# cloneofsimo/paint-with-words-sd

Measured on AMD Instinct MI355X. Metric: 512x512 images/sec (30 steps, CFG) SD1.5+PwW, higher is better.
Workload: dtype bf16

## Files before the change

__graft_entry__.py:

```python
import os
import sys

REPO = os.path.dirname(os.path.abspath(__file__))
PKG = os.path.join(REPO, "paint-with-words-sd_amd")
for p in (PKG, REPO, os.path.join(REPO, "tests")):
    if p not in sys.path:
        sys.path.insert(0, p)


def build():
    import build as pww_build
    lib = pww_build.build_lib(verbose=False)
    exe = pww_build.build_native_check()
    long_lib = pww_build.build_long()
    scope_lib = pww_build.build_scope()
    import pww_hip
    import paint_with_words
    handle = pww_hip.load_library()
    missing = [n for n in pww_hip.EXPORTS if not hasattr(handle, n)]
    assert not missing, "libpww_hip.so lacks %s" % missing
    from pww_hip import _lib
    long_handle = _lib.load_long()
    missing = [n for n in _lib.LONG_EXPORTS if not hasattr(long_handle, n)]
    assert not missing, "libpww_hip_long.so lacks %s" % missing
    scope_handle = _lib.load_scope()
    assert scope_handle is not None, "%s was not built" % scope_lib
    missing = [n for n in _lib.SCOPE_EXPORTS if not hasattr(scope_handle, n)]
    assert not missing, "libpww_hip_scope.so lacks %s" % missing
    print("built %s (ABI %d), %s (ABI %d), %s (ABI %d) and %s" % (lib, handle.pww_version(), long_lib, long_handle.pww_long_version(),
                                                                  scope_lib, scope_handle.pww_scope_version(), exe))


def smoke():
    import math
    import numpy as np
    import torch
    import pww_hip
    from oracle import pww_oracle as O
    import pww_cases as cases

    assert torch.cuda.is_available(), "smoke() needs a HIP device"
    dev = torch.device("cuda:0")
    print("device arch:", pww_hip.device_arch())

    case = cases.make_attention_case("sd15_n1024")
    dtype = torch.float16
    mod = case["attn_cross"].to(dev, dtype)
    hidden = case["hidden"].to(dev, dtype)
    wf = lambda w, sigma, qk: 0.4 * w * math.log(1 + sigma) * qk.max()
    ctx = {"CONTEXT_TENSOR": case["ctx"].to(dev, dtype), "CROSS_ATTENTION_WEIGHT_1024": case["w"].to(dev),
           "SIGMA": torch.tensor(7.84), "WEIGHT_FUNCTION": wf}
    y = pww_hip.inj_forward(mod, hidden, ctx).float().cpu()
    mod_ref = case["attn_cross"].to("cpu", dtype).float()
    ctx_ref = {"CONTEXT_TENSOR": case["ctx"].to(dtype).float(), "CROSS_ATTENTION_WEIGHT_1024": case["w"],
               "SIGMA": torch.tensor(7.84), "WEIGHT_FUNCTION": wf}
    ref = O.inj_forward(mod_ref, case["hidden"].to(dtype).float(), ctx_ref)
    err = (y - ref).abs().max().item() / ref.abs().max().item()
    print("cross-attention + PwW bias: max err / max|O| = %.3e" % err)
    assert err < 5e-3, err

    import paint_with_words as pw
    from PIL import Image
    tools = cases.build_tools("tiny", dtype=dtype, device=dev)
# ... 24 lines not shown
```

paint-with-words-sd_amd/build.py:

```python
import os
import subprocess
import sys

HERE = os.path.dirname(os.path.abspath(__file__))
REPO = os.path.dirname(HERE)
CSRC = os.path.join(HERE, "csrc")
LIB = os.path.join(HERE, "pww_hip", "libpww_hip.so")
LIB_EXPERIMENTS = os.path.join(HERE, "pww_hip", "libpww_hip_experiments.so")
LIB_LONG = os.path.join(HERE, "pww_hip", "libpww_hip_long.so")
LIB_SCOPE = os.path.join(HERE, "pww_hip", "libpww_hip_scope.so")
UNITS = [("pww_api.hip", [], ""), ("pww_attn.hip", [], ""), ("pww_cross.hip", [], ""), ("pww_cross_lean.hip", [], ""), ("pww_reduce.hip", [], ""),
         ("pww_mask.hip", [], ""), ("pww_qproj.hip", [], ""), ("pww_norm.hip", [], ""), ("pww_blocks.hip", [], ""), ("pww_conv.hip", [], ""), ("pww_probs.hip", [], ""),
         ("pww_attn_inst.hip", ["-DPWW_INST_F16"], ".f16"), ("pww_attn_inst.hip", ["-DPWW_INST_BF16"], ".bf16"),
         ("pww_cross_inst.hip", ["-DPWW_INST_F16", "-DPWW_INST_NW=2"], ".f16.nw2"), ("pww_cross_inst.hip", ["-DPWW_INST_F16", "-DPWW_INST_NW=4"], ".f16.nw4"),
         ("pww_cross_inst.hip", ["-DPWW_INST_BF16", "-DPWW_INST_NW=2"], ".bf16.nw2"), ("pww_cross_inst.hip", ["-DPWW_INST_BF16", "-DPWW_INST_NW=4"], ".bf16.nw4")]
EXPERIMENT_UNITS = [("pww_cross_out.hip", [], "")]
LONG_UNITS = [("pww_long.hip", ["-fvisibility=hidden"], "")]
LONG_HEADERS = ["pww_common.h", "pww_tile.h", "pww_attn_core.h", "pww_cross_tile.h", os.path.join(REPO, "include", "pww_hip.h"), os.path.join(REPO, "include", "pww_hip_long.h")]
SCOPE_UNITS = [("pww_scope.hip", ["-fvisibility=hidden"], "")]
SCOPE_HEADERS = ["pww_common.h", "pww_tile.h", "pww_attn_core.h", "pww_cross_tile.h", os.path.join(REPO, "include", "pww_hip.h"), os.path.join(REPO, "include", "pww_hip_scope.h")]
SOURCES = sorted({u[0] for u in UNITS + EXPERIMENT_UNITS})
HEADERS = ["pww_common.h", "pww_tile.h", "pww_attn_core.h", "pww_attn_kernel.h", "pww_cross_tile.h", "pww_cross_kernel.h", os.path.join(REPO, "include", "pww_hip.h")]
HIPCC = os.environ.get("HIPCC", "/opt/rocm/bin/hipcc")
FLAGS = ["--offload-arch=gfx950", "-O3", "-std=c++17", "-fPIC", "-Wall",
         "-Wno-unused-function", "-mllvm", "-amdgpu-kernarg-preload-count=16"]


PER_FILE_FLAGS = {"pww_mask.hip": ["-ffp-contract=off"]}


def _newer(target, deps):
    if not os.path.exists(target):
        return True
    t = os.path.getmtime(target)
    return any(os.path.getmtime(d) > t for d in deps)


def _deps():
    return ([os.path.join(CSRC, s) for s in SOURCES] + [h if os.path.isabs(h) else os.path.join(CSRC, h) for h in HEADERS] + [__file__])


def _build(lib, units, defines, objdir, verbose, jobs=None):
    os.makedirs(objdir, exist_ok=True)
    order = sorted(units, key=lambda u: {"pww_cross_inst.hip": 0, "pww_attn_inst.hip": 1, "pww_cross_lean.hip": 2}.get(u[0], 3))
    jobs = jobs or max(2, min(len(order), (os.cpu_count() or 4)))
    pending, running, objs = list(order), [], []
    while pending or running:
        while pending and len(running) < jobs:
            src, defs, suffix = pending.pop(0)
            o = os.path.join(objdir, src + suffix + ".o")
            objs.append(o)
            cmd = [HIPCC] + FLAGS + defines + defs + PER_FILE_FLAGS.get(src, []) + ["-c", os.path.join(CSRC, src), "-o", o]
            if verbose:
# ... 7 lines not shown
            raise RuntimeError("hipcc failed: %s\n%s" % (" ".join(cmd), out))
        if verbose and out.strip():
            print(out)
    subprocess.run([HIPCC, "--offload-arch=gfx950", "-shared", "-fPIC", "-s"] + sorted(objs) + ["-o", lib], check=True)
    return lib


def build_lib(force=False, verbose=False):
    if not force and not _newer(LIB, _deps()):
        return LIB
    return _build(LIB, UNITS, [], os.path.join(HERE, "build"), verbose)


def build_experiments(force=False, verbose=False):
    if not force and not _newer(LIB_EXPERIMENTS, _deps()):
        return LIB_EXPERIMENTS
    return _build(LIB_EXPERIMENTS, UNITS + EXPERIMENT_UNITS, ["-DPWW_EXPERIMENTS=1"], os.path.join(HERE, "build", "experiments"), verbose)


def build_long(force=False, verbose=False):
    deps = [os.path.join(CSRC, u[0]) for u in LONG_UNITS] + [h if os.path.isabs(h) else os.path.join(CSRC, h) for h in LONG_HEADERS] + [__file__]
    if not force and not _newer(LIB_LONG, deps):
        return LIB_LONG
    return _build(LIB_LONG, LONG_UNITS, [], os.path.join(HERE, "build", "long"), verbose)


def build_scope(force=False, verbose=False):
    deps = [os.path.join(CSRC, u[0]) for u in SCOPE_UNITS] + [h if os.path.isabs(h) else os.path.join(CSRC, h) for h in SCOPE_HEADERS] + [__file__]
    if not force and not _newer(LIB_SCOPE, deps):
        return LIB_SCOPE
    return _build(LIB_SCOPE, SCOPE_UNITS, [], os.path.join(HERE, "build", "scope"), verbose)


def _build_check(exe, lib, libname, defines, force):
    src = os.path.join(REPO, "tests", "native", "attn_check.cpp")
    if not force and not _newer(exe, [src, lib, os.path.join(REPO, "include", "pww_hip.h")]):
        return exe
    cmd = [HIPCC, "--offload-arch=gfx950", "-O2", "-std=c++17"] + defines + [src, "-o", exe, "-L" + os.path.dirname(lib), "-l" + libname,
                                                                              "-Wl,-rpath,$ORIGIN/../../paint-with-words-sd_amd/pww_hip"]
    subprocess.run(cmd, check=True)
    return exe


def build_native_check(force=False):
    return _build_check(os.path.join(REPO, "tests", "native", "attn_check"), build_lib(), "pww_hip", [], force)


def build_native_check_experiments(force=False):
    return _build_check(os.path.join(REPO, "tests", "native", "attn_check_experiments"), build_experiments(), "pww_hip_experiments", ["-DPWW_EXPERIMENTS=1"], force)


if __name__ == "__main__":
    force = "--force" in sys.argv
    print(build_lib(force=force, verbose=True))
    print(build_native_check(force=force))
    print(build_long(force=force, verbose=True))
    print(build_scope(force=force, verbose=True))
    if "--experiments" in sys.argv:
        print(build_experiments(force=force, verbose=True))
        print(build_native_check_experiments(force=force))
```

paint-with-words-sd_amd/pww_hip/_lib.py:

```python
import ctypes
import os

_HERE = os.path.dirname(os.path.abspath(__file__))
LIB_PATH = os.environ.get("PWW_HIP_LIB", os.path.join(_HERE, "libpww_hip.so"))
EXPERIMENTS_LIB_PATH = os.environ.get("PWW_HIP_EXPERIMENTS_LIB", os.path.join(_HERE, "libpww_hip_experiments.so"))

LONG_LIB_PATH = os.environ.get("PWW_HIP_LONG_LIB", os.path.join(_HERE, "libpww_hip_long.so"))

SCOPE_LIB_PATH = os.environ.get("PWW_HIP_SCOPE_LIB", os.path.join(_HERE, "libpww_hip_scope.so"))

PWW_OK, PWW_EINVAL, PWW_ENOTSUP, PWW_EHIP = 0, -22, -95, -5
MIN_VERSION = 126
DTYPE_F16, DTYPE_BF16 = 0, 1
LAYOUT_NCHW, LAYOUT_NHWC = 0, 1
ACT_NONE, ACT_SILU = 0, 1
MAX_HEAD_DIM = 160

EXPORTS = ("pww_version", "pww_has_experiments", "pww_last_error", "pww_device_arch", "pww_self_attn_fwd", "pww_cross_attn_fwd",
           "pww_cross_attn_fwd_stat", "pww_cross_attn_fwd_stat_ex",
           "pww_qk_reduce", "pww_mask_build", "pww_mask_build_rgb", "pww_mask_build_f32", "pww_resize_tokens", "pww_gauss_blur", "pww_inpaint_prep", "pww_cfg_combine", "pww_store_f32",
           "pww_workspace_bytes", "pww_profile_arm", "pww_profile_elapsed_us", "pww_profile_reset", "pww_debug_timeline", "pww_debug_path_counts",
           "pww_qproj_stat", "pww_qproj_parts", "pww_cross_attn_fwd_parts", "pww_mask_build_f32_levels", "pww_qk_parts", "pww_qk_parts_count",
           "pww_group_norm_fwd", "pww_group_norm_workspace_bytes", "pww_add_layer_norm", "pww_add_layer_norm_bias", "pww_geglu", "pww_bias_residual",
           "pww_conv3x3_workspace_bytes", "pww_conv3x3_fwd", "pww_cross_attn_probs")
EXPERIMENT_EXPORTS = ("pww_cross_attn_fwd_fused", "pww_cross_attn_fwd_fused_ex", "pww_cross_fused_workspace_bytes", "pww_cross_fused_state_bytes",
                      "pww_cross_attn_fwd_parts_out", "pww_cross_attn_out_supported")


LONG_EXPORTS = ("pww_long_version", "pww_long_last_error", "pww_long_qk_parts", "pww_long_qk_parts_count", "pww_long_cross_attn_fwd_parts",
                "pww_long_cross_attn_probs", "pww_long_profile_arm", "pww_long_profile_elapsed_us")
LONG_MIN_VERSION = 100
LONG_MIN_KEYS, LONG_MAX_KEYS = 129, 256


SCOPE_EXPORTS = ("pww_scope_version", "pww_scope_last_error", "pww_scope_head_parts_count", "pww_scope_head_parts", "pww_scope_cross_attn_fwd")
SCOPE_MIN_VERSION = 100
SCOPE_HEAD, SCOPE_ROW = 1, 2


class AttnDesc(ctypes.Structure):
    _fields_ = [("dtype", ctypes.c_int32), ("B", ctypes.c_int32), ("H", ctypes.c_int32), ("N", ctypes.c_int32),
                ("M", ctypes.c_int32), ("D", ctypes.c_int32),
                ("q_stride", ctypes.c_int64 * 3), ("k_stride", ctypes.c_int64 * 3),
                ("v_stride", ctypes.c_int64 * 3), ("o_stride", ctypes.c_int64 * 3),
                ("scale", ctypes.c_float), ("bias_stride", ctypes.c_int64 * 4)]


class CrossOpts(ctypes.Structure):
    _fields_ = [("size", ctypes.c_uint32), ("bias_cols", ctypes.c_int32), ("coeff_scalar_dev", ctypes.c_void_p),
                ("bias_compact", ctypes.c_void_p), ("col_idx", ctypes.c_void_p), ("R", ctypes.c_int32), ("gated_images", ctypes.c_int32),
                ("compact_stride", ctypes.c_int64 * 2), ("col_idx_stride", ctypes.c_int64)]


class QprojDesc(ctypes.Structure):
    _fields_ = [("dtype", ctypes.c_int32), ("B", ctypes.c_int32), ("N", ctypes.c_int32), ("Cin", ctypes.c_int32), ("H", ctypes.c_int32),
                ("D", ctypes.c_int32), ("M", ctypes.c_int32), ("x_stride", ctypes.c_int64 * 2), ("q_stride", ctypes.c_int64 * 2),
                ("k_stride", ctypes.c_int64 * 2)]


class GnDesc(ctypes.Structure):
    _fields_ = [("dtype", ctypes.c_int32), ("layout", ctypes.c_int32), ("B", ctypes.c_int32), ("C", ctypes.c_int32), ("HW", ctypes.c_int32),
                ("G", ctypes.c_int32), ("eps", ctypes.c_float), ("act", ctypes.c_int32), ("add_stride", ctypes.c_int32), ("_pad", ctypes.c_int32)]


class LnDesc(ctypes.Structure):
    _fields_ = [("dtype", ctypes.c_int32), ("C", ctypes.c_int32), ("rows", ctypes.c_int64), ("a_stride", ctypes.c_int64), ("x_stride", ctypes.c_int64),
                ("s_stride", ctypes.c_int64), ("y_stride", ctypes.c_int64), ("eps", ctypes.c_float), ("_pad", ctypes.c_int32)]


class ConvDesc(ctypes.Structure):
    _fields_ = [("size", ctypes.c_uint32), ("dtype", ctypes.c_int32), ("B", ctypes.c_int32), ("Hin", ctypes.c_int32), ("Win", ctypes.c_int32),
                ("Cin", ctypes.c_int32), ("Cout", ctypes.c_int32), ("stride", ctypes.c_int32), ("upsample", ctypes.c_int32), ("tile_n", ctypes.c_int32),
                ("splitk", ctypes.c_int32), ("_pad", ctypes.c_int32)]


class ProbsDesc(ctypes.Structure):
    _fields_ = [("size", ctypes.c_uint32), ("images", ctypes.c_int32), ("accumulate", ctypes.c_int32), ("weight", ctypes.c_float),
                ("out_stride", ctypes.c_int64 * 2)]


class Region(ctypes.Structure):
    _fields_ = [("r", ctypes.c_uint8), ("g", ctypes.c_uint8), ("b", ctypes.c_uint8), ("_pad", ctypes.c_uint8),
                ("strength", ctypes.c_float)]


class PwwHipError(RuntimeError):
    pass


_lib = None
_exp = None


def _bind(lib, experiments):
    vp, i32, i64, f32 = ctypes.c_void_p, ctypes.c_int32, ctypes.c_int64, ctypes.c_float
    lib.pww_version.restype = ctypes.c_int
    if lib.pww_version() // 100 != 1 or lib.pww_version() < MIN_VERSION:
        raise PwwHipError("libpww_hip ABI version %d.%02d is not 1.x >= 1.%02d (rebuild: python paint-with-words-sd_amd/build.py)"
                          % (lib.pww_version() // 100, lib.pww_version() % 100, MIN_VERSION % 100))
    lib.pww_last_error.restype = ctypes.c_char_p
    lib.pww_device_arch.argtypes = [ctypes.c_char_p, ctypes.c_size_t]
    lib.pww_self_attn_fwd.argtypes = [vp, vp, vp, vp, ctypes.POINTER(AttnDesc), vp]
    lib.pww_cross_attn_fwd.argtypes = [vp, vp, vp, vp, vp, vp, ctypes.POINTER(AttnDesc), vp]
    lib.pww_cross_attn_fwd_stat.argtypes = [vp, vp, vp, vp, vp, vp, i32, ctypes.c_double, f32, vp, ctypes.POINTER(AttnDesc), vp]
    lib.pww_cross_attn_fwd_stat_ex.argtypes = [vp, vp, vp, vp, vp, vp, i32, ctypes.c_double, f32, vp, ctypes.POINTER(AttnDesc),
                                               ctypes.POINTER(CrossOpts), vp]
# ... 145 lines not shown


def load_scope():
    global _scope
    if _scope is not None:
        return _scope
    if not os.path.isfile(SCOPE_LIB_PATH):
        return None
    hint = "(rebuild: python paint-with-words-sd_amd/build.py)"
    try:
        lib = ctypes.CDLL(SCOPE_LIB_PATH)
        lib.pww_scope_version.restype = ctypes.c_int
        version = lib.pww_scope_version()
    except (OSError, AttributeError) as e:
        raise PwwHipError("libpww_hip_scope.so at %s cannot be loaded: %s %s" % (SCOPE_LIB_PATH, e, hint))
    if version // 100 != 1 or version < SCOPE_MIN_VERSION:
        raise PwwHipError("libpww_hip_scope ABI version %d is not 1.x >= %d %s" % (version, SCOPE_MIN_VERSION, hint))
    missing = [n for n in SCOPE_EXPORTS if not hasattr(lib, n)]
    if missing:
        raise PwwHipError("libpww_hip_scope.so at %s lacks %s %s" % (SCOPE_LIB_PATH, missing, hint))
    vp, i32, f32 = ctypes.c_void_p, ctypes.c_int32, ctypes.c_float
    lib.pww_scope_last_error.restype = ctypes.c_char_p
    lib.pww_last_error = lib.pww_scope_last_error
    lib.pww_scope_head_parts_count.argtypes = [ctypes.POINTER(AttnDesc)]
    lib.pww_scope_head_parts_count.restype = ctypes.c_int32
    lib.pww_scope_head_parts.argtypes = [vp, vp, vp, ctypes.POINTER(AttnDesc), i32, vp, ctypes.c_size_t, vp]
    lib.pww_scope_head_parts.restype = ctypes.c_int
    lib.pww_scope_cross_attn_fwd.argtypes = [vp, vp, vp, vp, vp, i32, i32, f32, vp, ctypes.POINTER(AttnDesc), vp, i32, vp, ctypes.POINTER(CrossOpts), vp]
    lib.pww_scope_cross_attn_fwd.restype = ctypes.c_int
    _scope = lib
    return _scope


class experiments:

    def __enter__(self):
        global _lib
        load()
        self._prev = _lib
        _lib = load_experiments()
        return _lib

    def __exit__(self, *exc):
        global _lib
        _lib = self._prev
        return False


def check(rc, what, lib=None):
    if rc != PWW_OK:
        msg = (lib or load()).pww_last_error().decode("utf-8", "replace")
        raise PwwHipError("%s failed (rc=%d): %s" % (what, rc, msg))


def device_arch():
    buf = ctypes.create_string_buffer(64)
    check(load().pww_device_arch(buf, 64), "pww_device_arch")
    return buf.value.decode()
```

paint-with-words-sd_amd/pww_hip/blocks.py:

```python
import os
import types
import warnings

import torch
import torch.nn as nn
import torch.nn.functional as F

from . import ops

FUSED_NORM = os.environ.get("PWW_FUSED_NORM", "1") != "0"
BATCHED_TEMB = os.environ.get("PWW_BATCHED_TEMB", "1") != "0"
FOLD_CONV_BIAS = os.environ.get("PWW_FOLD_CONV_BIAS", "1") != "0"
CONV1X1_AS_LINEAR = os.environ.get("PWW_CONV1X1_AS_LINEAR", "1") != "0"
FUSE_FF_RESIDUAL = os.environ.get("PWW_FUSE_FF_RESIDUAL", "0") == "1"
CONV3X3 = os.environ.get("PWW_CONV3X3", "1") != "0"


_STATS = {k: [0, 0] for k in ("group_norm", "resnet_block", "transformer_block", "geglu", "conv1x1", "conv3x3")}
_UNRATED = ("conv1x1", "conv3x3")
_warned = set()


def stats():
    out = {k: {"fused": v[0], "declined": v[1]} for k, v in _STATS.items()}
    rated = [v for k, v in _STATS.items() if k not in _UNRATED]
    tot = sum(v[0] + v[1] for v in rated)
    out["hit_rate"] = (sum(v[0] for v in rated) / tot) if tot else None
    return out


def reset_stats():
    for v in _STATS.values():
        v[0] = v[1] = 0


def _count(op, fused, x=None, reason=None):
    _STATS[op][0 if fused else 1] += 1
    if not fused and FUSED_NORM and torch.is_tensor(x) and x.is_cuda and x.dtype in (torch.float16, torch.bfloat16):
        key = (op, reason)
        if key not in _warned:
            _warned.add(key)
            warnings.warn("pww_hip.blocks: %s call on a HIP %s tensor handed to the stock op (%s); pww_hip.blocks.stats() counts them"
                          % (op, str(x.dtype).split(".")[-1], reason or "shape / dtype the kernels do not take"), stacklevel=3)


def _why_not(x):
    if torch.is_autocast_enabled():
        return "torch.autocast is on: the norms run in fp32 there"
    if torch.is_grad_enabled() and torch.is_tensor(x) and x.requires_grad:
        return "autograd is recording: the kernels are forward-only"
    return None

# ... 176 lines not shown
    _STATS["conv1x1"][1] += 1
    return self._pww_orig_forward(x, *args, **kwargs)


def _is_conv1x1(m):
    return (isinstance(m, nn.Conv2d) and type(m).forward is nn.Conv2d.forward and m.kernel_size == (1, 1) and m.stride == (1, 1) and m.padding == (0, 0)
            and m.dilation == (1, 1) and m.groups == 1 and m.padding_mode == "zeros")


def _ln_takes(x, norm):
    return (FUSED_NORM and torch.is_tensor(x) and x.is_cuda and x.dtype in (torch.float16, torch.bfloat16) and x.dim() >= 2
            and len(norm.normalized_shape) == 1 and x.shape[-1] == norm.normalized_shape[0] and x.shape[-1] % 8 == 0 and x.shape[-1] <= 2048
            and (norm.weight is None or norm.weight.dtype == x.dtype) and not torch.is_autocast_enabled()
            and not (torch.is_grad_enabled() and (x.requires_grad or (norm.weight is not None and norm.weight.requires_grad))))


def _transformer_block_covered(m):
    return (all(isinstance(getattr(m, n, None), nn.LayerNorm) for n in ("norm1", "norm2", "norm3")) and hasattr(m, "attn1") and hasattr(m, "attn2")
            and hasattr(m, "ff") and not getattr(m, "only_cross_attention", False))


def _transformer_block_forward(self, *args, **kwargs):
    covered = 1 <= len(args) <= 2 and set(kwargs) <= {"context", "timestep"} and kwargs.get("timestep") is None and not (len(args) == 2 and "context" in kwargs)
    hidden_states = args[0] if args else None
    if not covered or not _ln_takes(hidden_states, self.norm1):
        _count("transformer_block", False, hidden_states, ("a call beyond (hidden_states, context, timestep=None): %d positional, keywords %s" % (len(args), sorted(kwargs)))
               if not covered else _why_not(hidden_states))
        return self._pww_orig_forward(*args, **kwargs)
    context = args[1] if len(args) == 2 else kwargs.get("context")
    _count("transformer_block", True)
    h = hidden_states
    n = ops.add_layer_norm(h, self.norm1.weight, self.norm1.bias, self.norm1.eps)
    h, n = ops.add_layer_norm(h, self.norm2.weight, self.norm2.bias, self.norm2.eps, a=self.attn1(n))
    lin = _ff_output_linear(self.ff) if FUSE_FF_RESIDUAL else None
    if lin is not None and lin.weight.dtype == h.dtype:
        h, n = ops.add_layer_norm(h, self.norm3.weight, self.norm3.bias, self.norm3.eps, a=self.attn2(n, context=context), post_bias=lin.bias)
        g = self.ff.net[0](n)
        return torch.addmm(h.reshape(-1, h.shape[-1]), g.reshape(-1, g.shape[-1]), lin.weight.t()).view(h.shape)
    h, n = ops.add_layer_norm(h, self.norm3.weight, self.norm3.bias, self.norm3.eps, a=self.attn2(n, context=context))
    return self.ff(n) + h


def _ff_output_linear(ff):
    net = getattr(ff, "net", None)
    if net is None or len(net) != 3 or type(ff).__name__ != "FeedForward" or "forward" in ff.__dict__:
        return None
    owner = next((c for c in type(ff).__mro__ if "forward" in c.__dict__), None)
    if owner is None or owner.__name__ != "FeedForward":
        return None
    act, drop, lin = net[0], net[1], net[2]
    if act.__class__.__name__ != "GEGLU" or not isinstance(drop, nn.Dropout) or (drop.training and drop.p > 0):
        return None
    if type(lin) is not nn.Linear or lin.bias is None or lin._forward_hooks or lin._forward_pre_hooks or "forward" in lin.__dict__ or ff._forward_hooks or ff._forward_pre_hooks:
        return None
    return lin


def _geglu_forward(self, x, *args, **kwargs):
    if args or kwargs:
        _count("geglu", False, x, "arguments beyond (hidden_states): %s" % (sorted(kwargs) or len(args)))
        return self._pww_orig_forward(x, *args, **kwargs)
    h = self.proj(x)
    if FUSED_NORM and h.is_cuda and h.dtype in (torch.float16, torch.bfloat16) and h.shape[-1] % 16 == 0 and not torch.is_autocast_enabled() \
            and not (torch.is_grad_enabled() and h.requires_grad):
        _count("geglu", True)
        return ops.geglu(h)
    _count("geglu", False, h, _why_not(h))
    a, gate = h.chunk(2, dim=-1)
    return a * F.gelu(gate)


def install_blocks(unet):
    n_res = n_gn = 0
    owned = set()
    plans = {}
    for m in unet.modules():
        if m.__class__.__name__ == "ResnetBlock2D" and _resnet_covered(m):
            if "_pww_orig_forward" not in m.__dict__:
                m.__dict__["_pww_orig_forward"] = m.forward
                m.forward = types.MethodType(_resnet_forward, m)
                lin = getattr(m, "time_emb_proj", None)
                if BATCHED_TEMB and isinstance(lin, nn.Linear):
                    m.__dict__["_pww_temb_slot"] = plans.setdefault(lin.in_features, TembProjections()).register(m)
            owned.update((id(m.norm1), id(m.norm2), id(m.conv1), id(m.conv2)))
            n_res += 1
    for m in unet.modules():
        name, fwd = m.__class__.__name__, None
        if isinstance(m, nn.GroupNorm) and id(m) not in owned:
            fwd = _group_norm_forward
            n_gn += 1
        elif name == "BasicTransformerBlock" and _transformer_block_covered(m):
            fwd = _transformer_block_forward
        elif name == "GEGLU" and isinstance(getattr(m, "proj", None), nn.Linear):
            fwd = _geglu_forward
# ... 20 lines not shown
```

paint-with-words-sd_amd/pww_hip/ops.py:

```python
import ctypes

import torch

from . import _lib
from ._lib import AttnDesc, CrossOpts, ProbsDesc, QprojDesc, Region, PwwHipError

_DT = {torch.float16: _lib.DTYPE_F16, torch.bfloat16: _lib.DTYPE_BF16}


def _stream():
    return ctypes.c_void_p(torch.cuda.current_stream().cuda_stream)


def _ptr(t):
    return ctypes.c_void_p(t.data_ptr()) if t is not None else ctypes.c_void_p(0)


def _require_gpu(*tensors):
    for t in tensors:
        if t is not None and not t.is_cuda:
            raise PwwHipError("pww_hip ops need tensors on a HIP device (got %s); there is no CPU path" % t.device)


def _rows_ok(t):
# ... 856 lines not shown
        return False
    B, C, H, W = x.shape
    Cout = weight.shape[0]
    return (tuple(weight.shape[1:]) == (C, 3, 3) and C % 64 == 0 and Cout % 64 == 0 and stride in (1, 2) and not (upsample and stride != 1)
            and x.is_contiguous(memory_format=torch.channels_last) and x.data_ptr() % 16 == 0
            and B * H * W * C < 2 ** 31 // 4)


def conv3x3(x, weight, bias=None, residual=None, stride=1, upsample=False, tile_n=0, splitk=0):
    _require_gpu(x, weight, bias, residual)
    if not conv3x3_takes(x, weight, stride, upsample):
        raise PwwHipError("conv3x3: needs a channels_last float16/bfloat16 x with Cin, Cout multiples of 64 and a 3 x 3 weight of its dtype")
    B, C, H, W = x.shape
    Cout = weight.shape[0]
    Hv, Wv = H << int(bool(upsample)), W << int(bool(upsample))
    Ho, Wo = (Hv - 1) // stride + 1, (Wv - 1) // stride + 1
    w = _khwc_weight(weight)
    if bias is not None and (bias.dtype != x.dtype or tuple(bias.shape) != (Cout,)):
        raise PwwHipError("conv3x3: bias must be a %s [%d]" % (x.dtype, Cout))
    if bias is not None:
        bias = bias.contiguous()
    if residual is not None:
        if tuple(residual.shape) != (B, Cout, Ho, Wo) or residual.dtype != x.dtype:
            raise PwwHipError("conv3x3: residual must be a %s %s" % (x.dtype, (B, Cout, Ho, Wo)))
        residual = residual.contiguous(memory_format=torch.channels_last)
    d = _lib.ConvDesc(ctypes.sizeof(_lib.ConvDesc), _DT[x.dtype], B, H, W, C, Cout, int(stride), int(bool(upsample)), int(tile_n), int(splitk), 0)
    lib = _lib.load()
    y = torch.empty((B, Cout, Ho, Wo), dtype=x.dtype, device=x.device, memory_format=torch.channels_last)
    nbytes = int(lib.pww_conv3x3_workspace_bytes(ctypes.byref(d)))
    ws = torch.empty(nbytes // 4, dtype=torch.float32, device=x.device) if nbytes else None
    with torch.cuda.device(x.device):
        _lib.check(lib.pww_conv3x3_fwd(_ptr(x), _ptr(w), _ptr(bias), _ptr(residual), _ptr(y), ctypes.byref(d), _ptr(ws), nbytes, _stream()), "pww_conv3x3_fwd")
    return y
```

Baseline: 5.016.

## Add MFMA linear kernel with fused GEGLU and bias-residual epilogues for FF

```diff
diff --git a/__graft_entry__.py b/__graft_entry__.py
--- a/__graft_entry__.py
+++ b/__graft_entry__.py
@@ -14,6 +14,7 @@
     exe = pww_build.build_native_check()
     long_lib = pww_build.build_long()
     scope_lib = pww_build.build_scope()
+    linear_lib = pww_build.build_linear()
     import pww_hip
     import paint_with_words
     handle = pww_hip.load_library()
@@ -27,8 +28,12 @@
     assert scope_handle is not None, "%s was not built" % scope_lib
     missing = [n for n in _lib.SCOPE_EXPORTS if not hasattr(scope_handle, n)]
     assert not missing, "libpww_hip_scope.so lacks %s" % missing
-    print("built %s (ABI %d), %s (ABI %d), %s (ABI %d) and %s" % (lib, handle.pww_version(), long_lib, long_handle.pww_long_version(),
-                                                                  scope_lib, scope_handle.pww_scope_version(), exe))
+    linear_handle = _lib.load_linear()
+    missing = [n for n in _lib.LINEAR_EXPORTS if not hasattr(linear_handle, n)]
+    assert not missing, "libpww_hip_linear.so lacks %s" % missing
+    print("built %s (ABI %d), %s (ABI %d), %s (ABI %d), %s (ABI %d) and %s" % (lib, handle.pww_version(), long_lib, long_handle.pww_long_version(),
+                                                                              scope_lib, scope_handle.pww_scope_version(), linear_lib,
+                                                                              linear_handle.pww_linear_version(), exe))
 
 
 def smoke():
diff --git a/include/pww_hip_linear.h b/include/pww_hip_linear.h
--- /dev/null
+++ b/include/pww_hip_linear.h
@@ -0,0 +1,35 @@
+#ifndef PWW_HIP_LINEAR_H
+#define PWW_HIP_LINEAR_H
+
+#include "pww_hip.h"
+
+#ifdef __cplusplus
+extern "C" {
+#endif
+
+#define PWW_LINEAR_VERSION 100
+
+int pww_linear_version(void);
+const char *pww_linear_last_error(void);
+
+#define PWW_LINEAR_NONE 0
+#define PWW_LINEAR_BIAS 1
+#define PWW_LINEAR_BIAS_RESIDUAL 2
+#define PWW_LINEAR_BIAS_GEGLU 3
+typedef struct pww_linear_desc {
+    uint32_t size;
+    int32_t dtype;
+    int32_t M, N, K;
+    int32_t epilogue;
+    int64_t x_stride, y_stride, r_stride;
+    int32_t tile_n, splitk;
+} pww_linear_desc_t;
+size_t pww_linear_workspace_bytes(const pww_linear_desc_t *desc);
+int pww_linear_fwd(const void *x, const void *w, const void *bias, const void *residual, void *y, const pww_linear_desc_t *desc, void *workspace,
+                   size_t workspace_bytes, void *stream);
+
+#ifdef __cplusplus
+}
+#endif
+
+#endif
diff --git a/paint-with-words-sd_amd/build.py b/paint-with-words-sd_amd/build.py
--- a/paint-with-words-sd_amd/build.py
+++ b/paint-with-words-sd_amd/build.py
@@ -9,6 +9,7 @@
 LIB_EXPERIMENTS = os.path.join(HERE, "pww_hip", "libpww_hip_experiments.so")
 LIB_LONG = os.path.join(HERE, "pww_hip", "libpww_hip_long.so")
 LIB_SCOPE = os.path.join(HERE, "pww_hip", "libpww_hip_scope.so")
+LIB_LINEAR = os.path.join(HERE, "pww_hip", "libpww_hip_linear.so")
 UNITS = [("pww_api.hip", [], ""), ("pww_attn.hip", [], ""), ("pww_cross.hip", [], ""), ("pww_cross_lean.hip", [], ""), ("pww_reduce.hip", [], ""),
          ("pww_mask.hip", [], ""), ("pww_qproj.hip", [], ""), ("pww_norm.hip", [], ""), ("pww_blocks.hip", [], ""), ("pww_conv.hip", [], ""), ("pww_probs.hip", [], ""),
          ("pww_attn_inst.hip", ["-DPWW_INST_F16"], ".f16"), ("pww_attn_inst.hip", ["-DPWW_INST_BF16"], ".bf16"),
@@ -19,6 +20,8 @@
 LONG_HEADERS = ["pww_common.h", "pww_tile.h", "pww_attn_core.h", "pww_cross_tile.h", os.path.join(REPO, "include", "pww_hip.h"), os.path.join(REPO, "include", "pww_hip_long.h")]
 SCOPE_UNITS = [("pww_scope.hip", ["-fvisibility=hidden"], "")]
 SCOPE_HEADERS = ["pww_common.h", "pww_tile.h", "pww_attn_core.h", "pww_cross_tile.h", os.path.join(REPO, "include", "pww_hip.h"), os.path.join(REPO, "include", "pww_hip_scope.h")]
+LINEAR_UNITS = [("pww_linear.hip", ["-fvisibility=hidden"], "")]
+LINEAR_HEADERS = ["pww_common.h", os.path.join(REPO, "include", "pww_hip.h"), os.path.join(REPO, "include", "pww_hip_linear.h")]
 SOURCES = sorted({u[0] for u in UNITS + EXPERIMENT_UNITS})
 HEADERS = ["pww_common.h", "pww_tile.h", "pww_attn_core.h", "pww_attn_kernel.h", "pww_cross_tile.h", "pww_cross_kernel.h", os.path.join(REPO, "include", "pww_hip.h")]
 HIPCC = os.environ.get("HIPCC", "/opt/rocm/bin/hipcc")
@@ -92,6 +95,13 @@
     return _build(LIB_SCOPE, SCOPE_UNITS, [], os.path.join(HERE, "build", "scope"), verbose)
 
 
+def build_linear(force=False, verbose=False):
+    deps = [os.path.join(CSRC, u[0]) for u in LINEAR_UNITS] + [h if os.path.isabs(h) else os.path.join(CSRC, h) for h in LINEAR_HEADERS] + [__file__]
+    if not force and not _newer(LIB_LINEAR, deps):
+        return LIB_LINEAR
+    return _build(LIB_LINEAR, LINEAR_UNITS, [], os.path.join(HERE, "build", "linear"), verbose)
+
+
 def _build_check(exe, lib, libname, defines, force):
     src = os.path.join(REPO, "tests", "native", "attn_check.cpp")
     if not force and not _newer(exe, [src, lib, os.path.join(REPO, "include", "pww_hip.h")]):
@@ -116,6 +126,7 @@
     print(build_native_check(force=force))
     print(build_long(force=force, verbose=True))
     print(build_scope(force=force, verbose=True))
+    print(build_linear(force=force, verbose=True))
     if "--experiments" in sys.argv:
         print(build_experiments(force=force, verbose=True))
         print(build_native_check_experiments(force=force))
diff --git a/paint-with-words-sd_amd/csrc/pww_linear.hip b/paint-with-words-sd_amd/csrc/pww_linear.hip
--- /dev/null
+++ b/paint-with-words-sd_amd/csrc/pww_linear.hip
@@ -0,0 +1,351 @@
+#include <string.h>
+#include "pww_common.h"
+#include "../../include/pww_hip_linear.h"
+
+#define PWW_LINEAR_API extern "C" __attribute__((visibility("default")))
+
+namespace pww {
+
+static thread_local char g_linear_err[512] = "";
+
+void set_error(const char *fmt, ...) {
+    va_list ap;
+    va_start(ap, fmt);
+    vsnprintf(g_linear_err, sizeof(g_linear_err), fmt, ap);
+    va_end(ap);
+}
+
+int check_hip(hipError_t e, const char *what) {
+    if (e == hipSuccess) return PWW_OK;
+    set_error("%s: %s (%s)", what, hipGetErrorString(e), hipGetErrorName(e));
+    return PWW_EHIP;
+}
+
+bool arch_ok() {
+    static thread_local int cached = -1;
+    if (cached < 0) {
+        int dev = 0;
+        hipDeviceProp_t prop;
+        if (check_hip(hipGetDevice(&dev), "hipGetDevice") || check_hip(hipGetDeviceProperties(&prop, dev), "hipGetDeviceProperties")) return false;
+        cached = strncmp(prop.gcnArchName, "gfx950", 6) == 0 && (prop.gcnArchName[6] == 0 || prop.gcnArchName[6] == ':') ? 1 : 0;
+    }
+    if (!cached) set_error("libpww_hip_linear is built for gfx950 (MI355X) only");
+    return cached == 1;
+}
+
+bool profile_take(hipEvent_t *, hipEvent_t *, hipStream_t) { return false; }
+
+namespace {
+
+constexpr int LN_BM = 128, LN_THREADS = 256;
+constexpr int LN_PF = 2;
+
+__device__ __forceinline__ f32x4 mfma16(f16x8 a, f16x8 b, f32x4 c) { return __builtin_amdgcn_mfma_f32_16x16x32_f16(a, b, c, 0, 0, 0); }
+__device__ __forceinline__ f32x4 mfma16(bf16x8 a, bf16x8 b, f32x4 c) { return __builtin_amdgcn_mfma_f32_16x16x32_bf16(a, b, c, 0, 0, 0); }
+
+struct LinCold {
+    const void *bias, *residual;
+    long ys, rs;
+    int nsplit, nslab, mode, inner;
+};
+
+__device__ __forceinline__ int xcd_remap(int orig, int nwg) {
+    const int xcd = orig & 7, q = nwg >> 3, r = nwg & 7;
+    return (xcd < r ? xcd * (q + 1) : r * (q + 1) + (xcd - r) * q) + (orig >> 3);
+}
+
+template <typename T> __device__ __forceinline__ float rnd(float v) { return (float)(T)v; }
+
+template <typename T>
+__device__ __forceinline__ void epilogue4(const f32x4 &a, const LinCold &cold, T *y, int m, int n) {
+    typedef typename Vec<T>::v4 V4;
+    V4 o;
+#pragma unroll
+    for (int j = 0; j < 4; ++j) o[j] = (T)a[j];
+    if (cold.mode >= PWW_LINEAR_BIAS) {
+        const V4 b = *reinterpret_cast<const V4 *>(reinterpret_cast<const T *>(cold.bias) + n);
+#pragma unroll
+        for (int j = 0; j < 4; ++j) o[j] = (T)((float)o[j] + (float)b[j]);
+    }
+    if (cold.mode == PWW_LINEAR_BIAS_RESIDUAL) {
+        const V4 r = *reinterpret_cast<const V4 *>(reinterpret_cast<const T *>(cold.residual) + (long)m * cold.rs + n);
+#pragma unroll
+        for (int j = 0; j < 4; ++j) o[j] = (T)((float)r[j] + (float)o[j]);
+    }
+    *reinterpret_cast<V4 *>(y + (long)m * cold.ys + n) = o;
+}
+
+template <typename T>
+__device__ __forceinline__ void geglu4(const f32x4 &av, const f32x4 &ag, const LinCold &cold, T *y, int m, int j0) {
+    typedef typename Vec<T>::v4 V4;
+    const V4 bv = *reinterpret_cast<const V4 *>(reinterpret_cast<const T *>(cold.bias) + j0);
+    const V4 bg = *reinterpret_cast<const V4 *>(reinterpret_cast<const T *>(cold.bias) + cold.inner + j0);
+    V4 o;
+#pragma unroll
+    for (int j = 0; j < 4; ++j) {
+        const float hv = rnd<T>(rnd<T>(av[j]) + (float)bv[j]);
+        const float g = rnd<T>(rnd<T>(ag[j]) + (float)bg[j]);
+        const float ge = rnd<T>(0.5f * g * (1.f + erff(g * 0.70710678118654752440f)));
+        o[j] = (T)(hv * ge);
+    }
+    *reinterpret_cast<V4 *>(y + (long)m * cold.ys + j0) = o;
+}
+
+template <typename T, int BN>
+__global__ void __launch_bounds__(LN_THREADS, 2) linear_kernel(const T *__restrict__ x, const T *__restrict__ w, void *out, int M, int N, int K, int xs,
+                                                               const LinCold cold) {
+    typedef typename Vec<T>::v8 V8;
+    constexpr int BM = LN_BM, PF = LN_PF, XL = BM * 8 / LN_THREADS, WL = BN * 8 / LN_THREADS, RM = 4, RN = BN / 32;
+    constexpr int XBYTES = BM * 128, STAGE = (BM + BN) * 128;
+    __shared__ __attribute__((aligned(16))) char lds[2 * STAGE];
+
+    const int tid = threadIdx.x, lane = tid & 63, wave = tid >> 6, wm = wave >> 1, wn = wave & 1;
+    const int ntm = (M + BM - 1) / BM;
+    const int bid = xcd_remap(blockIdx.x, gridDim.x);
+    const bool split = cold.nsplit > 1;
+    const bool geglu = cold.mode == PWW_LINEAR_BIAS_GEGLU;
+    const int tile = bid / cold.nsplit, ks = bid - tile * cold.nsplit;
+    const int tm = tile % ntm, tn = tile / ntm;
+    const int s_begin = (int)((long)ks * cold.nslab / cold.nsplit), s_end = (int)((long)(ks + 1) * cold.nslab / cold.nsplit);
+
+    const int c = tid & 7;
+    unsigned xoff[XL], woff[WL];
+#pragma unroll
+    for (int i = 0; i < XL; ++i) {
+        int m = tm * BM + (tid >> 3) + 32 * i;
+        m = m < M ? m : M - 1;
+        xoff[i] = (unsigned)(m * xs + c * 8);
+    }
+#pragma unroll
+    for (int j = 0; j < WL; ++j) {
+        const int t = (tid >> 3) + 32 * j;
+        const int u = t % (BN / 2);
+        const int row = geglu ? (u >= BN / 4 ? cold.inner : 0) + tn * (BN / 2) + (t / (BN / 2)) * (BN / 4) + u % (BN / 4) : tn * BN + t;
+        woff[j] = (unsigned)(row * K + c * 8);
+    }
+    const int swz = ((c ^ ((tid >> 3) & 7)) << 4);
+
+    u32x4 xr[PF][XL], wr[PF][WL];
+    const T *xnext = x + s_begin * 64, *wnext = w + s_begin * 64;
+    auto load = [&](int p) {
+#pragma unroll
+        for (int i = 0; i < XL; ++i) xr[p][i] = *reinterpret_cast<const u32x4 *>(xnext + xoff[i]);
+#pragma unroll
+        for (int j = 0; j < WL; ++j) wr[p][j] = *reinterpret_cast<const u32x4 *>(wnext + woff[j]);
+        xnext += 64;
+        wnext += 64;
+    };
+    auto store = [&](int p, int buf) {
+        char *base = lds + buf * STAGE;
+#pragma unroll
+        for (int i = 0; i < XL; ++i) *reinterpret_cast<u32x4 *>(base + ((tid >> 3) + 32 * i) * 128 + swz) = xr[p][i];
+#pragma unroll
+        for (int j = 0; j < WL; ++j) *reinterpret_cast<u32x4 *>(base + XBYTES + ((tid >> 3) + 32 * j) * 128 + swz) = wr[p][j];
+    };
+
+    f32x4 acc[RN][RM];
+#pragma unroll
+    for (int r = 0; r < RN; ++r)
+#pragma unroll
+        for (int i = 0; i < RM; ++i) acc[r][i] = f32x4{0.f, 0.f, 0.f, 0.f};
+
+    const int fr = lane & 15, fq = lane >> 4;
+    auto compute = [&](int buf) {
+        const char *bx = lds + buf * STAGE, *bw = bx + XBYTES;
+#pragma unroll
+        for (int kk = 0; kk < 2; ++kk) {
+            V8 xf[RM], wf[RN];
+#pragma unroll
+            for (int q = 0; q < RM; ++q) {
+                const int row = wm * 64 + q * 16 + fr;
+                xf[q] = *reinterpret_cast<const V8 *>(bx + row * 128 + (((kk * 4 + fq) ^ (row & 7)) << 4));
+            }
+#pragma unroll
+            for (int r = 0; r < RN; ++r) {
+                const int row = wn * (BN / 2) + r * 16 + fr;
+                wf[r] = *reinterpret_cast<const V8 *>(bw + row * 128 + (((kk * 4 + fq) ^ (row & 7)) << 4));
+            }
+#pragma unroll
+            for (int r = 0; r < RN; ++r)
+#pragma unroll
+                for (int q = 0; q < RM; ++q) acc[r][q] = mfma16(wf[r], xf[q], acc[r][q]);
+        }
+    };
+
+    const int n = s_end - s_begin;
+    load(0);
+#pragma unroll
+    for (int p = 1; p < PF; ++p)
+        if (p < n) load(p);
+    store(0, 0);
+    __syncthreads();
+    int i = 0;
+    for (; i + 2 * PF <= n; i += PF) {
+#pragma unroll
+        for (int p = 0; p < PF; ++p) {
+            load(p);
+            compute((i + p) & 1);
+            store((p + 1) % PF, (i + p + 1) & 1);
+            __syncthreads();
+        }
+    }
+#pragma unroll
+    for (int t = 0; t < 2 * PF - 1; ++t) {
+        if (i + t < n) {
+            if (i + t + PF < n) load(t % PF);
+            compute((i + t) & 1);
+            if (i + t + 1 < n) store((t + 1) % PF, (i + t + 1) & 1);
+            __syncthreads();
+        }
+    }
+
+#pragma unroll
+    for (int i = 0; i < RM; ++i) {
+        const int m = tm * BM + wm * 64 + i * 16 + fr;
+        if (m >= M) continue;
+        if (split) {
+#pragma unroll
+            for (int r = 0; r < RN; ++r) {
+                const int col = geglu ? (r >= RN / 2 ? cold.inner : 0) + tn * (BN / 2) + wn * (BN / 4) + (r % (RN / 2)) * 16 + fq * 4
+                                      : tn * BN + wn * (BN / 2) + r * 16 + fq * 4;
+                *reinterpret_cast<f32x4 *>(reinterpret_cast<float *>(out) + ((long)ks * M + m) * N + col) = acc[r][i];
+            }
+        } else if (geglu) {
+#pragma unroll
+            for (int r = 0; r < RN / 2; ++r)
+                geglu4<T>(acc[r][i], acc[r + RN / 2][i], cold, reinterpret_cast<T *>(out), m, tn * (BN / 2) + wn * (BN / 4) + r * 16 + fq * 4);
+        } else {
+#pragma unroll
+            for (int r = 0; r < RN; ++r) epilogue4<T>(acc[r][i], cold, reinterpret_cast<T *>(out), m, tn * BN + wn * (BN / 2) + r * 16 + fq * 4);
+        }
+    }
+}
+
+template <typename T>
+__global__ void __launch_bounds__(256) linear_fold_kernel(const float *__restrict__ ws, T *y, long n4, int N, long MN, const LinCold cold) {
+    const long q = (long)blockIdx.x * 256 + threadIdx.x;
+    if (q >= n4) return;
+    const bool geglu = cold.mode == PWW_LINEAR_BIAS_GEGLU;
+    const int nout = geglu ? cold.inner : N;
+    const long o4 = q * 4;
+    const int m = (int)(o4 / nout), n = (int)(o4 - (long)m * nout);
+    const float *p = ws + (long)m * N + n;
+    f32x4 a = *reinterpret_cast<const f32x4 *>(p);
+    for (int s = 1; s < cold.nsplit; ++s) a += *reinterpret_cast<const f32x4 *>(p + s * MN);
+    if (geglu) {
+        f32x4 g = *reinterpret_cast<const f32x4 *>(p + cold.inner);
+        for (int s = 1; s < cold.nsplit; ++s) g += *reinterpret_cast<const f32x4 *>(p + s * MN + cold.inner);
+        geglu4<T>(a, g, cold, y, m, n);
+    } else {
+        epilogue4<T>(a, cold, y, m, n);
+    }
+}
+
+struct LinTune { int M, N, nslab, geglu, bn, nsplit; };
+constexpr LinTune LIN_TUNED[] = {
+    {8192, 2560, 5, 1, 64, 1}, {2048, 5120, 10, 1, 64, 1}, {512, 10240, 20, 1, 64, 1}, {128, 10240, 20, 1, 64, 1},
+    {8192, 320, 20, 0, 64, 1}, {8192, 320, 5, 0, 64, 1}, {2048, 640, 40, 0, 128, 3}, {2048, 640, 10, 0, 64, 1},
+    {512, 1280, 80, 0, 64, 3}, {512, 1280, 20, 0, 64, 2}, {128, 1280, 80, 0, 64, 5}, {128, 1280, 20, 0, 64, 4},
+};
+
+struct LinPlan {
+    int bn, nsplit, nslab, ntiles, nout;
+    long xs, ys, rs;
+};
+
+bool plan_linear(const pww_linear_desc_t *d, LinPlan *p) {
+    if (!d || d->size < sizeof(pww_linear_desc_t)) { set_error("linear: descriptor missing or older than this library (size %u)", d ? d->size : 0u); return false; }
+    const int e = d->epilogue;
+    const bool geglu = e == PWW_LINEAR_BIAS_GEGLU;
+    if ((d->dtype != PWW_DTYPE_F16 && d->dtype != PWW_DTYPE_BF16) || d->M < 1 || d->K < 64 || d->K % 64 != 0 || d->N < 64 || d->N % 64 != 0
+        || e < PWW_LINEAR_NONE || e > PWW_LINEAR_BIAS_GEGLU || (geglu && d->N % 128 != 0)) {
+        set_error("linear: unsupported (dtype %d M %d N %d K %d epilogue %d): K and N multiples of 64, GEGLU's inner = N / 2 a multiple of 64", d->dtype,
+                  d->M, d->N, d->K, e);
+        return false;
+    }
+    p->nout = geglu ? d->N / 2 : d->N;
+    p->xs = d->x_stride ? d->x_stride : d->K;
+    p->ys = d->y_stride ? d->y_stride : p->nout;
+    p->rs = d->r_stride ? d->r_stride : p->nout;
+    if (p->xs < d->K || p->ys < p->nout || p->rs < p->nout || ((p->xs | p->ys | p->rs) & 7)) {
+        set_error("linear: row strides must cover their rows and be multiples of 8 elements (x %ld y %ld r %ld)", p->xs, p->ys, p->rs);
+        return false;
+    }
+    if ((long)d->M * p->xs >= (1L << 31) || (long)d->N * d->K >= (1L << 31) || (long)d->M * d->N >= (1L << 31)) { set_error("linear: tensor of 2^31 elements or more"); return false; }
+    p->nslab = d->K / 64;
+    const LinTune *tuned = nullptr;
+    for (const LinTune &t : LIN_TUNED)
+        if (t.M == d->M && t.N == d->N && t.nslab == p->nslab && t.geglu == (int)geglu) tuned = &t;
+    p->bn = d->tile_n ? d->tile_n : tuned ? tuned->bn : (d->N % 128 == 0 ? 128 : 64);
+    if ((p->bn != 64 && p->bn != 128) || d->N % p->bn != 0) { set_error("linear: tile_n %d does not divide N %d", d->tile_n, d->N); return false; }
+    p->ntiles = (d->M + LN_BM - 1) / LN_BM * (d->N / p->bn);
+    int ns = d->splitk;
+    if (ns <= 0 && tuned && p->bn == tuned->bn) ns = tuned->nsplit;
+    if (ns <= 0) {
+        ns = (480 + p->ntiles / 2) / p->ntiles;
+        if (ns > p->nslab / 4) ns = p->nslab / 4;
+        if (ns < 1) ns = 1;
+    }
+    if (ns > p->nslab || ns > 64) { set_error("linear: split %d exceeds the %d K-slabs (or 64)", ns, p->nslab); return false; }
+    p->nsplit = ns;
+    return true;
+}
+
+template <typename T>
+int linear_launch(const LinPlan &p, const pww_linear_desc_t *d, const void *x, const void *w, const void *bias, const void *residual, void *y, void *ws,
+                  hipStream_t stream) {
+    LinCold cold{bias, residual, p.ys, p.rs, p.nsplit, p.nslab, d->epilogue, d->N / 2};
+    const T *xt = static_cast<const T *>(x), *wt = static_cast<const T *>(w);
+    const dim3 grid(p.ntiles * p.nsplit), block(LN_THREADS);
+    void *out = p.nsplit == 1 ? y : ws;
+    if (p.bn == 128) launch_timed(linear_kernel<T, 128>, grid, block, 0, stream, xt, wt, out, d->M, d->N, d->K, (int)p.xs, cold);
+    else launch_timed(linear_kernel<T, 64>, grid, block, 0, stream, xt, wt, out, d->M, d->N, d->K, (int)p.xs, cold);
+    if (p.nsplit == 1) return check_hip(hipGetLastError(), "linear launch");
+    const long MN = (long)d->M * d->N, n4 = (long)d->M * p.nout / 4;
+    launch_timed(linear_fold_kernel<T>, dim3((unsigned)((n4 + 255) / 256)), dim3(256), 0, stream, static_cast<const float *>(ws), static_cast<T *>(y), n4,
+                 d->N, MN, cold);
+    return check_hip(hipGetLastError(), "linear fold launch");
+}
+
+bool al16(const void *a) { return (reinterpret_cast<uintptr_t>(a) & 15) == 0; }
+
+}
+
+size_t linear_workspace_bytes(const pww_linear_desc_t *d) {
+    LinPlan p;
+    if (!plan_linear(d, &p)) return 0;
+    return p.nsplit > 1 ? (size_t)p.nsplit * d->M * d->N * sizeof(float) : 0;
+}
+
+int linear_fwd(const void *x, const void *w, const void *bias, const void *residual, void *y, const pww_linear_desc_t *d, void *workspace,
+               size_t workspace_bytes, hipStream_t stream) {
+    LinPlan p;
+    if (!plan_linear(d, &p)) return PWW_ENOTSUP;
+    if (!x || !w || !y) { set_error("linear: x, w and y are required"); return PWW_EINVAL; }
+    if ((d->epilogue >= PWW_LINEAR_BIAS && !bias) || (d->epilogue == PWW_LINEAR_BIAS_RESIDUAL && !residual)) {
+        set_error("linear: epilogue %d needs its bias%s", d->epilogue, d->epilogue == PWW_LINEAR_BIAS_RESIDUAL ? " and residual" : "");
+        return PWW_EINVAL;
+    }
+    if (!al16(x) || !al16(w) || !al16(y) || (reinterpret_cast<uintptr_t>(bias) & 7) || (reinterpret_cast<uintptr_t>(residual) & 7)) {
+        set_error("linear: x, w, y must be 16-byte aligned, bias and residual 8-byte aligned");
+        return PWW_EINVAL;
+    }
+    const size_t need = p.nsplit > 1 ? (size_t)p.nsplit * d->M * d->N * sizeof(float) : 0;
+    if (need && (!workspace || !al16(workspace) || workspace_bytes < need)) {
+        set_error("linear: split %d needs a 16-byte aligned workspace of %zu bytes (got %zu)", p.nsplit, need, workspace_bytes);
+        return PWW_EINVAL;
+    }
+    if (!arch_ok()) return PWW_ENOTSUP;
+    if (d->dtype == PWW_DTYPE_F16) return linear_launch<f16>(p, d, x, w, bias, residual, y, workspace, stream);
+    return linear_launch<bf16>(p, d, x, w, bias, residual, y, workspace, stream);
+}
+
+}
+
+PWW_LINEAR_API int pww_linear_version(void) { return PWW_LINEAR_VERSION; }
+PWW_LINEAR_API const char *pww_linear_last_error(void) { return pww::g_linear_err; }
+PWW_LINEAR_API size_t pww_linear_workspace_bytes(const pww_linear_desc_t *desc) { return pww::linear_workspace_bytes(desc); }
+PWW_LINEAR_API int pww_linear_fwd(const void *x, const void *w, const void *bias, const void *residual, void *y, const pww_linear_desc_t *desc,
+                                  void *workspace, size_t workspace_bytes, void *stream) {
+    return pww::linear_fwd(x, w, bias, residual, y, desc, workspace, workspace_bytes, static_cast<hipStream_t>(stream));
+}
diff --git a/paint-with-words-sd_amd/pww_hip/_lib.py b/paint-with-words-sd_amd/pww_hip/_lib.py
--- a/paint-with-words-sd_amd/pww_hip/_lib.py
+++ b/paint-with-words-sd_amd/pww_hip/_lib.py
@@ -8,12 +8,15 @@
 LONG_LIB_PATH = os.environ.get("PWW_HIP_LONG_LIB", os.path.join(_HERE, "libpww_hip_long.so"))
 
 SCOPE_LIB_PATH = os.environ.get("PWW_HIP_SCOPE_LIB", os.path.join(_HERE, "libpww_hip_scope.so"))
+
+LINEAR_LIB_PATH = os.environ.get("PWW_HIP_LINEAR_LIB", os.path.join(_HERE, "libpww_hip_linear.so"))
 
 PWW_OK, PWW_EINVAL, PWW_ENOTSUP, PWW_EHIP = 0, -22, -95, -5
 MIN_VERSION = 126
 DTYPE_F16, DTYPE_BF16 = 0, 1
 LAYOUT_NCHW, LAYOUT_NHWC = 0, 1
 ACT_NONE, ACT_SILU = 0, 1
+LINEAR_NONE, LINEAR_BIAS, LINEAR_BIAS_RESIDUAL, LINEAR_BIAS_GEGLU = 0, 1, 2, 3
 MAX_HEAD_DIM = 160
 
 EXPORTS = ("pww_version", "pww_has_experiments", "pww_last_error", "pww_device_arch", "pww_self_attn_fwd", "pww_cross_attn_fwd",
@@ -38,6 +41,10 @@
 SCOPE_HEAD, SCOPE_ROW = 1, 2
 
 
+LINEAR_EXPORTS = ("pww_linear_version", "pww_linear_last_error", "pww_linear_workspace_bytes", "pww_linear_fwd")
+LINEAR_MIN_VERSION = 100
+
+
 class AttnDesc(ctypes.Structure):
     _fields_ = [("dtype", ctypes.c_int32), ("B", ctypes.c_int32), ("H", ctypes.c_int32), ("N", ctypes.c_int32),
                 ("M", ctypes.c_int32), ("D", ctypes.c_int32),
@@ -72,6 +79,12 @@
     _fields_ = [("size", ctypes.c_uint32), ("dtype", ctypes.c_int32), ("B", ctypes.c_int32), ("Hin", ctypes.c_int32), ("Win", ctypes.c_int32),
                 ("Cin", ctypes.c_int32), ("Cout", ctypes.c_int32), ("stride", ctypes.c_int32), ("upsample", ctypes.c_int32), ("tile_n", ctypes.c_int32),
                 ("splitk", ctypes.c_int32), ("_pad", ctypes.c_int32)]
+
+
+class LinearDesc(ctypes.Structure):
+    _fields_ = [("size", ctypes.c_uint32), ("dtype", ctypes.c_int32), ("M", ctypes.c_int32), ("N", ctypes.c_int32), ("K", ctypes.c_int32),
+                ("epilogue", ctypes.c_int32), ("x_stride", ctypes.c_int64), ("y_stride", ctypes.c_int64), ("r_stride", ctypes.c_int64),
+                ("tile_n", ctypes.c_int32), ("splitk", ctypes.c_int32)]
 
 
 class ProbsDesc(ctypes.Structure):
@@ -283,6 +296,36 @@
     return _scope
 
 
+_linear = None
+
+
+def load_linear():
+    global _linear
+    if _linear is not None:
+        return _linear
+    hint = "(rebuild: python paint-with-words-sd_amd/build.py)"
+    try:
+        lib = ctypes.CDLL(LINEAR_LIB_PATH)
+        lib.pww_linear_version.restype = ctypes.c_int
+        version = lib.pww_linear_version()
+    except (OSError, AttributeError) as e:
+        raise PwwHipError("libpww_hip_linear.so at %s cannot be loaded: %s %s" % (LINEAR_LIB_PATH, e, hint))
+    if version // 100 != 1 or version < LINEAR_MIN_VERSION:
+        raise PwwHipError("libpww_hip_linear ABI version %d is not 1.x >= %d %s" % (version, LINEAR_MIN_VERSION, hint))
+    missing = [n for n in LINEAR_EXPORTS if not hasattr(lib, n)]
+    if missing:
+        raise PwwHipError("libpww_hip_linear.so at %s lacks %s %s" % (LINEAR_LIB_PATH, missing, hint))
+    vp = ctypes.c_void_p
+    lib.pww_linear_last_error.restype = ctypes.c_char_p
+    lib.pww_last_error = lib.pww_linear_last_error
+    lib.pww_linear_workspace_bytes.argtypes = [ctypes.POINTER(LinearDesc)]
+    lib.pww_linear_workspace_bytes.restype = ctypes.c_size_t
+    lib.pww_linear_fwd.argtypes = [vp, vp, vp, vp, vp, ctypes.POINTER(LinearDesc), vp, ctypes.c_size_t, vp]
+    lib.pww_linear_fwd.restype = ctypes.c_int
+    _linear = lib
+    return _linear
+
+
 class experiments:
 
     def __enter__(self):
diff --git a/paint-with-words-sd_amd/pww_hip/blocks.py b/paint-with-words-sd_amd/pww_hip/blocks.py
--- a/paint-with-words-sd_amd/pww_hip/blocks.py
+++ b/paint-with-words-sd_amd/pww_hip/blocks.py
@@ -12,12 +12,12 @@
 BATCHED_TEMB = os.environ.get("PWW_BATCHED_TEMB", "1") != "0"
 FOLD_CONV_BIAS = os.environ.get("PWW_FOLD_CONV_BIAS", "1") != "0"
 CONV1X1_AS_LINEAR = os.environ.get("PWW_CONV1X1_AS_LINEAR", "1") != "0"
-FUSE_FF_RESIDUAL = os.environ.get("PWW_FUSE_FF_RESIDUAL", "0") == "1"
+LINEAR = os.environ.get("PWW_LINEAR", "1")
 CONV3X3 = os.environ.get("PWW_CONV3X3", "1") != "0"
 
 
-_STATS = {k: [0, 0] for k in ("group_norm", "resnet_block", "transformer_block", "geglu", "conv1x1", "conv3x3")}
-_UNRATED = ("conv1x1", "conv3x3")
+_STATS = {k: [0, 0] for k in ("group_norm", "resnet_block", "transformer_block", "geglu", "conv1x1", "conv3x3", "linear")}
+_UNRATED = ("conv1x1", "conv3x3", "linear")
 _warned = set()
 
 
@@ -260,12 +260,13 @@
     h = hidden_states
     n = ops.add_layer_norm(h, self.norm1.weight, self.norm1.bias, self.norm1.eps)
     h, n = ops.add_layer_norm(h, self.norm2.weight, self.norm2.bias, self.norm2.eps, a=self.attn1(n))
-    lin = _ff_output_linear(self.ff) if FUSE_FF_RESIDUAL else None
-    if lin is not None and lin.weight.dtype == h.dtype:
-        h, n = ops.add_layer_norm(h, self.norm3.weight, self.norm3.bias, self.norm3.eps, a=self.attn2(n, context=context), post_bias=lin.bias)
+    h, n = ops.add_layer_norm(h, self.norm3.weight, self.norm3.bias, self.norm3.eps, a=self.attn2(n, context=context))
+    lin = _ff_output_linear(self.ff) if LINEAR != "0" else None
+    if lin is not None:
         g = self.ff.net[0](n)
-        return torch.addmm(h.reshape(-1, h.shape[-1]), g.reshape(-1, g.shape[-1]), lin.weight.t()).view(h.shape)
-    h, n = ops.add_layer_norm(h, self.norm3.weight, self.norm3.bias, self.norm3.eps, a=self.attn2(n, context=context))
+        if _linear_route(g, lin.weight, lin.bias, "residual", residual=h):
+            return ops.linear(g, lin.weight, lin.bias, residual=h)
+        return lin(g) + h
     return self.ff(n) + h
 
 
@@ -282,12 +283,36 @@
     if type(lin) is not nn.Linear or lin.bias is None or lin._forward_hooks or lin._forward_pre_hooks or "forward" in lin.__dict__ or ff._forward_hooks or ff._forward_pre_hooks:
         return None
     return lin
+
+
+LINEAR_ROUTES = frozenset([
+    (8192, 320, 2560, "geglu"),
+    (2048, 640, 5120, "geglu"),
+    (512, 1280, 10240, "geglu"),
+    (128, 1280, 10240, "geglu"),
+    (512, 5120, 1280, "residual"),
+])
+
+
+def _linear_route(x, weight, bias, epilogue, residual=None):
+    ok = (LINEAR != "0" and FUSED_NORM and not torch.is_autocast_enabled() and torch.is_tensor(x) and bias is not None and bias.dtype == x.dtype
+          and not (torch.is_grad_enabled() and (x.requires_grad or weight.requires_grad)) and ops.linear_takes(x, weight, epilogue == "geglu", bias=bias, residual=residual)
+          and (LINEAR == "force" or (x.numel() // x.shape[-1], x.shape[-1], weight.shape[0], epilogue) in LINEAR_ROUTES))
+    _STATS["linear"][0 if ok else 1] += 1
+    return ok
+
+
+def _plain_linear(lin):
+    return type(lin) is nn.Linear and lin.bias is not None and not lin._forward_hooks and not lin._forward_pre_hooks and "forward" not in lin.__dict__
 
 
 def _geglu_forward(self, x, *args, **kwargs):
     if args or kwargs:
         _count("geglu", False, x, "arguments beyond (hidden_states): %s" % (sorted(kwargs) or len(args)))
         return self._pww_orig_forward(x, *args, **kwargs)
+    if _plain_linear(self.proj) and _linear_route(x, self.proj.weight, self.proj.bias, "geglu"):
+        _count("geglu", True)
+        return ops.linear(x, self.proj.weight, self.proj.bias, geglu=True)
     h = self.proj(x)
     if FUSED_NORM and h.is_cuda and h.dtype in (torch.float16, torch.bfloat16) and h.shape[-1] % 16 == 0 and not torch.is_autocast_enabled() \
             and not (torch.is_grad_enabled() and h.requires_grad):
diff --git a/paint-with-words-sd_amd/pww_hip/ops.py b/paint-with-words-sd_amd/pww_hip/ops.py
--- a/paint-with-words-sd_amd/pww_hip/ops.py
+++ b/paint-with-words-sd_amd/pww_hip/ops.py
@@ -912,3 +912,72 @@
     with torch.cuda.device(x.device):
         _lib.check(lib.pww_conv3x3_fwd(_ptr(x), _ptr(w), _ptr(bias), _ptr(residual), _ptr(y), ctypes.byref(d), _ptr(ws), nbytes, _stream()), "pww_conv3x3_fwd")
     return y
+
+
+def _linear_weight(weight):
+    if not torch.is_tensor(weight) or weight.dim() not in (2, 4) or (weight.dim() == 4 and tuple(weight.shape[2:]) != (1, 1)):
+        return None
+    w = weight.detach().reshape(weight.shape[0], weight.shape[1]) if weight.dim() == 4 else weight.detach()
+    return w if w.is_contiguous() and w.data_ptr() == weight.data_ptr() and w.data_ptr() % 16 == 0 else None
+
+
+def linear_takes(x, weight, geglu=False, bias=None, residual=None, out=None):
+    if not (torch.is_tensor(x) and x.is_cuda and x.dtype in _DT and x.dim() >= 2 and torch.is_tensor(weight) and weight.dtype == x.dtype):
+        return False
+    w = _linear_weight(weight)
+    if w is None or x.shape[-1] != w.shape[1] or x.numel() == 0 or _rows(x, "linear") is None:
+        return False
+    N, K = w.shape
+    rows, _, xs = _rows(x, "linear")
+    if not (K % 64 == 0 and N % (128 if geglu else 64) == 0 and rows * xs < 2 ** 31 and rows * N < 2 ** 31 and N * K < 2 ** 31):
+        return False
+    if bias is not None and not (torch.is_tensor(bias) and bias.is_cuda and bias.dtype == x.dtype and tuple(bias.shape) == (N,) and bias.is_contiguous()
+                                 and bias.data_ptr() % 8 == 0):
+        return False
+    shape = tuple(x.shape[:-1]) + (N // 2 if geglu else N,)
+    for t in (residual, out):
+        if t is not None and not (torch.is_tensor(t) and t.is_cuda and t.dtype == x.dtype and tuple(t.shape) == shape and _rows(t, "linear") is not None):
+            return False
+    return True
+
+
+def linear(x, weight, bias=None, residual=None, geglu=False, tile_n=0, splitk=0, out=None):
+    _require_gpu(x, weight, bias, residual, out)
+    if not linear_takes(x, weight, geglu):
+        raise PwwHipError("linear: needs a float16/bfloat16 [..., K] x with one row pitch and a dense [N, K] weight of its dtype, K and N multiples of 64%s"
+                          % (" (geglu: N / 2 a multiple of 64)" if geglu else ""))
+    w = _linear_weight(weight)
+    N, K = w.shape
+    M, _, xs = _rows(x, "linear")
+    nout = N // 2 if geglu else N
+    if (geglu or residual is not None) and bias is None:
+        raise PwwHipError("linear: the residual and GEGLU epilogues need the bias")
+    if geglu and residual is not None:
+        raise PwwHipError("linear: geglu and residual exclude each other")
+    if bias is not None:
+        if bias.dtype != x.dtype or tuple(bias.shape) != (N,):
+            raise PwwHipError("linear: bias must be a %s [%d]" % (x.dtype, N))
+        bias = bias.contiguous() if bias.data_ptr() % 8 == 0 else bias.clone(memory_format=torch.contiguous_format)
+    shape = tuple(x.shape[:-1]) + (nout,)
+    rs = 0
+    if residual is not None:
+        if tuple(residual.shape) != shape or residual.dtype != x.dtype:
+            raise PwwHipError("linear: residual must be a %s %s" % (x.dtype, shape))
+        r = _rows(residual, "linear")
+        if r is None:
+            residual = residual.contiguous()
+            r = _rows(residual, "linear")
+        rs = r[2]
+    if out is None:
+        out = torch.empty(shape, dtype=x.dtype, device=x.device)
+    elif tuple(out.shape) != shape or out.dtype != x.dtype or _rows(out, "linear") is None:
+        raise PwwHipError("linear: out must be a %s %s whose rows have one pitch" % (x.dtype, shape))
+    ys = _rows(out, "linear")[2]
+    epi = _lib.LINEAR_BIAS_GEGLU if geglu else _lib.LINEAR_BIAS_RESIDUAL if residual is not None else _lib.LINEAR_BIAS if bias is not None else _lib.LINEAR_NONE
+    d = _lib.LinearDesc(ctypes.sizeof(_lib.LinearDesc), _DT[x.dtype], M, N, K, epi, xs, ys, rs, int(tile_n), int(splitk))
+    lib = _lib.load_linear()
+    nbytes = int(lib.pww_linear_workspace_bytes(ctypes.byref(d)))
+    ws = torch.empty(nbytes // 4, dtype=torch.float32, device=x.device) if nbytes else None
+    with torch.cuda.device(x.device):
+        _lib.check(lib.pww_linear_fwd(_ptr(x), _ptr(w), _ptr(bias), _ptr(residual), _ptr(out), ctypes.byref(d), _ptr(ws), nbytes, _stream()), "pww_linear_fwd", lib)
+    return out
```

New measurement: 5.113, median of 6. 1.9% higher.
